# UWQuickstep/quickstep

Measured on AMD Instinct MI355X. Metric: probe+aggregate rows/s at TPC-H SF100 (Q1,Q3), higher is better.
Workload: dtype i32 keys / f64 sums

## Files before the change

quickstep_amd/capi.py:

```python
import ctypes as C
import os

import torch

from . import types as T

_HERE = os.path.dirname(os.path.abspath(__file__))
LIB_PATH = os.environ.get("QSX_LIB_PATH") or os.path.join(_HERE, "lib", "libqsx.so")


class QsxError(RuntimeError):
    def __init__(self, status, where):
        self.status = status
        msg = _lib.qsx_status_string(status).decode()
        detail = _lib.qsx_last_error().decode()
        super().__init__(f"{where}: {msg} ({status})" + (f" — {detail}" if detail and status in (T.ERR_HIP, T.ERR_COMM) else ""))


def _load():
    if not os.path.exists(LIB_PATH):
        raise ImportError(
            f"{LIB_PATH} is missing: build it with `python -c 'import __graft_entry__ as g; g.build()'` "
            "(or make -C quickstep_amd/csrc). There is no CPU fallback for the HIP execution kernel.")
    return C.CDLL(LIB_PATH)
# ... 120 lines not shown
    "qsx_agg_state_image_layout": (_int, [_vp, C.POINTER(_int), C.POINTER(_i64), C.POINTER(_i64), C.POINTER(_int), C.POINTER(_i32), _int]),
    "qsx_agg_state_import_merge": (_int, [_vp, _vp, _sz, _vp]),
    "qsx_agg_num_groups": (_int, [_vp, C.POINTER(_i64), _vp]),
    "qsx_agg_finalize": (_int, [_vp, _int, _int, _pp, _pp, _pp, _i64, _vp, _vp]),
    "qsx_lip_filter_create": (_int, [_int, _i64, _i64, _int, _pp]),
    "qsx_lip_filter_destroy": (_int, [_vp]),
    "qsx_lip_build": (_int, [_vp, _int, _vp, _i64, _vp, _vp]),
    "qsx_lip_build_from_join_table": (_int, [_vp, _vp, _i64, _vp]),
    "qsx_lip_probe": (_int, [_vp, _int, _vp, _i64, _vp, _vp, _vp, _vp]),
    "qsx_lip_build_blocks": (_int, [_vp, _int, _i64, C.POINTER(_i64), _pp, _pp, _vp]),
    "qsx_lip_probe_blocks": (_int, [_vp, _int, _i64, C.POINTER(_i64), _pp, _pp, _pp, _vp, _vp]),
    "qsx_lip_build_blocks_coded": (_int, [_vp, _int, _i64, C.POINTER(_i64), _pp, _vp, _pp, _vp]),
    "qsx_lip_probe_blocks_coded": (_int, [_vp, _int, _i64, C.POINTER(_i64), _pp, _vp, _pp, _pp, _vp, _vp]),
    "qsx_lip_filter_words": (_int, [_vp, _pp, C.POINTER(_i64)]),
    "qsx_comm_unique_id": (_int, [_vp]),
    "qsx_comm_create": (_int, [_int, _int, _vp, _pp]),
    "qsx_comm_destroy": (_int, [_vp]),
    "qsx_comm_rank": (_int, [_vp, C.POINTER(_int), C.POINTER(_int)]),
    "qsx_comm_agree": (_int, [_vp, _int, _vp]),
    "qsx_comm_synchronize": (_int, [_vp, _vp]),
    "qsx_comm_abort": (_int, [_vp]),
    "qsx_exchange_counts": (_int, [_vp, _vp, _vp, _vp]),
    "qsx_alltoallv": (_int, [_vp, _int, _vp, C.POINTER(_i64), _vp, C.POINTER(_i64), _vp]),
    "qsx_allgather": (_int, [_vp, _vp, _sz, _vp, _vp]),
    "qsx_bitmap_allreduce_or": (_int, [_vp, _vp, _i64, _vp]),
    "qsx_agg_reduce_scatter": (_int, [_vp, _vp, _vp]),
    "qsx_agg_allgather_merge": (_int, [_vp, _vp, _vp]),
    "qsx_agg_dense_partition_range": (_int, [_i64, _int, _int, C.POINTER(_i64), C.POINTER(_i64), C.POINTER(_i64), C.POINTER(_i64),
                                             C.POINTER(C.c_uint64), C.POINTER(C.c_uint64)]),
    "qsx_partition_workspace_bytes": (_sz, [_i64, _int]),
    "qsx_partition_scatter": (_int, [_int, _vp, _i64, _int, _int, _pp, C.POINTER(_i32), _pp, _vp, _vp, _sz, _vp]),
    "qsx_partition_blocks_workspace_bytes": (_sz, [_i64, _i64, _int]),
    "qsx_partition_scatter_blocks": (_int, [_int, _i64, C.POINTER(_i64), _pp, _int, _int, _pp, C.POINTER(_i32), _pp, _vp, _vp, _sz, _vp]),
}

for _name, (_res, _args) in _SIGNATURES.items():
    _fn = getattr(_lib, _name)
    _fn.restype = _res
    _fn.argtypes = _args

if _lib.qsx_abi_sizeof_agg_config() != C.sizeof(T.AggConfig):
    raise ImportError("quickstep_amd.types.AggConfig does not match qsx_agg_config_t of libqsx.so")

if _lib.qsx_abi_sizeof_sort_key() != C.sizeof(T.SortKey):
    raise ImportError("quickstep_amd.types.SortKey does not match qsx_sort_key_t of libqsx.so")

if _lib.qsx_abi_sizeof_case_desc() != C.sizeof(T.CaseDesc):
    raise ImportError("quickstep_amd.types.CaseDesc does not match qsx_case_desc_t of libqsx.so")

lib = _lib
EXPORTED = tuple(_SIGNATURES)


def _check(status, where):
    if status != T.OK:
        raise QsxError(status, where)


def trim_scratch():
    v = C.c_size_t()
    _check(_lib.qsx_trim_scratch(C.byref(v)), "qsx_trim_scratch")
    return v.value


def device_count():
    return _lib.qsx_device_count()


def current_device():
    v = C.c_int(-1)
    _check(_lib.qsx_current_device(C.byref(v)), "qsx_current_device")
    return v.value


def set_current_device(device):
    _check(_lib.qsx_set_current_device(int(device)), "qsx_set_current_device")


def _ptr(t):
    return None if t is None else C.c_void_p(t.data_ptr())


def _stream(stream=None):
    s = torch.cuda.current_stream() if stream is None else stream
    return C.c_void_p(s.cuda_stream)


_TORCH_TYPE = {torch.int32: T.INT, torch.int64: T.LONG, torch.float32: T.FLOAT, torch.float64: T.DOUBLE,
               torch.uint8: T.CHAR}
_C_SCALAR = {T.INT: C.c_int32, T.LONG: C.c_int64, T.FLOAT: C.c_float, T.DOUBLE: C.c_double}


def qsx_type_of(t):
    return _TORCH_TYPE[t.dtype]


def bitmap_words(n):
    return (n + 63) // 64


def new_bitmap(n, device):
    return torch.empty(max(bitmap_words(n), 1), dtype=torch.int64, device=device)


def _ptr_array(tensors):
    arr = (C.c_void_p * max(len(tensors), 1))()
# ... 1139 lines not shown
```

quickstep_amd/csrc/join.hip:

```cpp

#include "common.hpp"
#include "join_dense.hpp"
#include "join_lds.hpp"
#include "scan.hpp"

#include <atomic>
#include <cstdlib>
#include <vector>
#include <mutex>
#include <shared_mutex>
#include <type_traits>

namespace qsx {

constexpr int kJBlock = 256;
constexpr uint64_t kEmpty64 = ~0ull;
constexpr uint32_t kEmptyTid = 0xFFFFFFFFu;

struct alignas(16) LongEntry {
  int64_t key;
  uint32_t tid;
  uint32_t pad;
};

// ... 1202 lines not shown
  for (int64_t b = 0; b < num_blocks; ++b) {
    const int64_t last = base[b] + block_rows[b] - 1;
    for (int64_t seen = t->max_tid.load(); seen < last && !t->max_tid.compare_exchange_weak(seen, last);) {}
  }
  hipStream_t s = as_stream(stream);
  std::vector<long long> table;
  const long long groups = build_run_table(kBuildTile, num_blocks, block_rows, block_keys,
                                           reinterpret_cast<const void *const *>(block_filters), nullptr, base.data(), &table,
                                           coding != nullptr ? coding->block_code_width : nullptr,
                                           coding != nullptr ? coding->block_dictionaries : nullptr);
  if (groups < 0) return QSX_ERR_INVALID_ARGUMENT;
  const size_t bytes = table.size() * sizeof(long long);
  const long long *runs_dev = static_cast<const long long *>(staged_device_buffer(s, bytes));
  if (runs_dev == nullptr) return QSX_ERR_OUT_OF_MEMORY;
  rc = staged_upload(s, table.data(), bytes);
  if (rc != QSX_OK) return rc;
  std::shared_lock<std::shared_mutex> lock(t->mutex);
  if (t->dense) {
    const int dgrid = grid_for(groups, kDBlock / kWave);
    if (t->key_type == QSX_INT) {
      hipLaunchKernelGGL((dense_build_kernel<int32_t, true>), dim3(dgrid), dim3(kDBlock), 0, s, t->dense_view(),
                         static_cast<const int32_t *>(nullptr), total, 0, static_cast<const uint64_t *>(nullptr), t->entries_dev, runs_dev);
    } else {
      hipLaunchKernelGGL((dense_build_kernel<int64_t, true>), dim3(dgrid), dim3(kDBlock), 0, s, t->dense_view(),
                         static_cast<const int64_t *>(nullptr), total, 0, static_cast<const uint64_t *>(nullptr), t->entries_dev, runs_dev);
    }
  } else {
    const int grid = grid_for(groups, kJBlock / kWave);
    if (t->key_type == QSX_INT) {
      hipLaunchKernelGGL(build_runs_kernel<int32_t>, dim3(grid), dim3(kJBlock), 0, s, t->view(), runs_dev, t->entries_dev);
    } else {
      hipLaunchKernelGGL(build_runs_kernel<int64_t>, dim3(grid), dim3(kJBlock), 0, s, t->view(), runs_dev, t->entries_dev);
    }
  }
  QSX_CHECK_LAUNCH();
  mark_stream(t, s);
  return QSX_OK;
}

int qsx_join_build_blocks(qsx_join_table_t *t, int64_t num_blocks, const int64_t *block_rows, const void *const *block_keys,
                          const int32_t *block_base_tids, const uint64_t *const *block_filters, qsx_stream_t stream) {
  return join_build_blocks_impl(t, num_blocks, block_rows, block_keys, block_base_tids, block_filters, nullptr, stream);
}
int qsx_join_build_blocks_coded(qsx_join_table_t *t, int64_t num_blocks, const int64_t *block_rows, const void *const *block_keys,
                                const qsx_key_coding_t *coding, const int32_t *block_base_tids, const uint64_t *const *block_filters,
                                qsx_stream_t stream) {
  return join_build_blocks_impl(t, num_blocks, block_rows, block_keys, block_base_tids, block_filters, coding, stream);
}

}

static std::atomic<long long> g_compact_probes{0};
extern "C" long long qsx_debug_join_compact_probes(void) { return g_compact_probes.load(std::memory_order_relaxed); }
static bool lds_tables_enabled() {
  const char *e = getenv("QSX_JOIN_LDS");
  return e == nullptr || e[0] != '0';
}

static bool dense_two_pass(const uint64_t *filter) {
  const char *e = getenv("QSX_JOIN_TWO_PASS");
  if (e != nullptr && e[0] != '\0') return e[0] != '0';
  return filter != nullptr;
}

static void drop_cover(qsx_join_table *t) {
  std::lock_guard<std::mutex> lock(t->cover_mutex);
  t->cover_state = 0;
  t->cover_sig.clear();
}

constexpr int64_t kAdaptiveMinRows = 1 << 16;
static bool adaptive_enabled() {
  const char *e = getenv("QSX_JOIN_ADAPTIVE");
  return e == nullptr || e[0] != '0';
}

static bool sealed_pack(qsx_join_table *t, hipStream_t stream, unsigned long long *count_word = nullptr) {
  auto behind_the_pack = [&]() {
    if (t->pack_stream != stream && t->pack_event != nullptr && hipEventQuery(t->pack_event) != hipSuccess) {
      (void)hipGetLastError();
      (void)hipStreamWaitEvent(stream, t->pack_event, 0);
    }
  };
  int state = t->seal_state.load(std::memory_order_acquire);
  if (state == 2) {
    behind_the_pack();
    return false;
  }
  if (state != 0 || !adaptive_enabled()) return false;
  const uint64_t bytes4 = t->range * 4, bytes3 = t->range * 3;
  if (bytes4 <= (13ull << 18) || bytes3 > (36ull << 20) / 10 || t->max_tid.load() >= (1 << 23) - 2 || t->reserved >= (1 << 23) - 1) {
    return false;
  }
  std::lock_guard<std::mutex> lock(t->seal_mutex);
  state = t->seal_state.load(std::memory_order_acquire);
  if (state != 0) {
    if (state == 2) behind_the_pack();
    return false;
  }
  if (t->head3 == nullptr && device_malloc(&t->head3, static_cast<size_t>(bytes3) + 4) != hipSuccess) {
    (void)hipGetLastError();
    t->head3 = nullptr;
    t->seal_state.store(1, std::memory_order_release);
    return false;
  }
  if (t->pack_event == nullptr && hipEventCreateWithFlags(&t->pack_event, hipEventDisableTiming) != hipSuccess) {
// ... 159 lines not shown
    if (!ensure_scanned()) return nullptr;
    if (!compact_possible(t) || !read_control_words(t, stream, v, &any_key) || !seal_compact(t, v[2] != 0, stream) || !publish_seal(t, stream, 3)) {
      t->seal_state.store(1, std::memory_order_release);
    }
    return nullptr;
  }
  qsx_join_table *shadow = t->shadow;
  if (shadow != nullptr && (shadow->min_key != lo || shadow->range != span + 1 || shadow->ov_capacity < entries)) {
    (void)qsx_join_table_destroy(shadow);
    shadow = t->shadow = nullptr;
  }
  if (shadow == nullptr) {
    if (qsx_join_table_create_dense(t->key_type, lo, hi, 1, static_cast<int64_t>(entries), &shadow) != QSX_OK) {
      (void)hipGetLastError();
      return stays_hashed();
    }
    t->shadow = shadow;
  } else if (qsx_join_table_clear(shadow, reinterpret_cast<qsx_stream_t>(stream)) != QSX_OK) {
    return stays_hashed();
  }
  shadow->reserved = static_cast<int64_t>(entries);
  shadow->max_tid.store(t->max_tid.load());
  const TableView src = t->view();
  hipLaunchKernelGGL(dense_build_from_slots_kernel, dim3(grid_for(static_cast<int64_t>(src.num_slots()), kJBlock * 4)), dim3(kJBlock), 0, stream,
                     t->key_type == QSX_LONG ? 1 : 0, src, shadow->dense_view());
  if (hipGetLastError() != hipSuccess) return stays_hashed();
  if (seal_verify_enabled()) {
    int error = 0;
    if (hipStreamSynchronize(stream) != hipSuccess ||
        hipMemcpy(&error, shadow->entries_dev + 3, sizeof(error), hipMemcpyDeviceToHost) != hipSuccess || error != 0) {
      set_last_error("QSX_JOIN_SEAL_VERIFY: the shadow's build reported an error", hipErrorUnknown);
      return stays_hashed();
    }
  }
  if (!publish_seal(t, stream, 2)) return stays_hashed();
  return shadow;
}

template <int MODE, bool kRuns, bool kLds = true, int NLIP = 0>
static int launch_lds_dense_probe(qsx_join_table_t *t, const void *keys, int64_t n, int32_t probe_base_tid, const uint64_t *filter,
                                  int32_t *out_probe, int32_t *out_build, int64_t capacity, unsigned long long *count,
                                  uint64_t *out_bitmap, int anti, hipStream_t stream, const long long *runs_dev, int64_t tiles,
                                  const LipViews &lips = LipViews{}) {
  const size_t table_bytes = kLds ? ((static_cast<size_t>(t->range) * 4 + 15) & ~static_cast<size_t>(15)) : 0;
  auto launch = [&](auto key_tag) -> int {
    using KeyT = decltype(key_tag);
    auto kernel = &lds_dense_probe_kernel<KeyT, MODE, kRuns, kLds, NLIP>;
    if (table_bytes > 48 * 1024) {
      QSX_HIP_TRY(hipFuncSetAttribute(reinterpret_cast<const void *>(kernel), hipFuncAttributeMaxDynamicSharedMemorySize, 160 * 1024 - kLdsStaticBytes));
    }
    const int sub = kLds ? kLdsSub : kLdsSubGlobal, per_cu = kLds ? 1 : 2;
    const int64_t units = (tiles + sub - 1) / sub;
    const int grid = static_cast<int>(units < static_cast<int64_t>(per_cu) * kCUs ? units : static_cast<int64_t>(per_cu) * kCUs);
    hipLaunchKernelGGL(kernel, dim3(grid), dim3(kLdsBlock), table_bytes, stream, t->dense_view(), static_cast<const KeyT *>(keys), n, probe_base_tid,
                       filter, out_probe, out_build, capacity, count, out_bitmap, anti, runs_dev, lips);
    QSX_CHECK_LAUNCH();
    return QSX_OK;
  };
  return t->key_type == QSX_INT ? launch(int32_t{}) : launch(int64_t{});
}

static bool one_pass_enabled() {
  const char *e = getenv("QSX_JOIN_ONE_PASS");
  return e == nullptr || e[0] != '0';
}

template <int MODE, bool kRuns = false>
static int launch_probe(qsx_join_table_t *t, const void *keys, int64_t n, int32_t probe_base_tid,
                        const uint64_t *filter, int32_t *out_probe, int32_t *out_build,
                        int64_t capacity, int64_t *out_count, uint64_t *out_bitmap, int anti,
                        hipStream_t stream, const long long *runs_dev = nullptr, int64_t run_tiles = 0) {
  static_assert(kDenseTile == kProbeTile, "one run table serves both table kinds");
  if (!t->dense && n != 0) {
    qsx_join_table *shadow = sealed_shadow(t, stream, n);
    if (shadow != nullptr) {
      return launch_probe<MODE, kRuns>(shadow, keys, n, probe_base_tid, filter, out_probe, out_build, capacity, out_count, out_bitmap,
                                       anti, stream, runs_dev, run_tiles);
    }
    if (!t->scanned.load(std::memory_order_acquire)) {
      set_last_error("the scan in front of a hashed table's first probe could not be issued", hipErrorUnknown);
      return QSX_ERR_HIP;
    }
  }
  const bool zeroed = n != 0 && t->dense && sealed_pack(t, stream, reinterpret_cast<unsigned long long *>(out_count));
  if (out_count != nullptr && !zeroed) QSX_HIP_TRY(hipMemsetAsync(out_count, 0, sizeof(int64_t), stream));
  if (n == 0) return QSX_OK;
  std::shared_lock<std::shared_mutex> lock(t->mutex);
  if (t->dense) {
    const int64_t tiles = kRuns ? run_tiles : (n + kDenseTile - 1) / kDenseTile;
    const int64_t limit = 8 * kCUs;
    const int dgrid = static_cast<int>(tiles < limit ? tiles : limit);
    unsigned long long *dcount = reinterpret_cast<unsigned long long *>(out_count);
    if constexpr (MODE == 0 || MODE == 1 || MODE == 2) {
      const bool two_pass = MODE == 0 && dense_two_pass(filter);
      if (!two_pass && lds_tables_enabled() && t->range <= static_cast<uint64_t>(kLdsDenseMaxWords) && n >= 32 * static_cast<int64_t>(t->range) &&
          n >= (1 << 18)) {
        return launch_lds_dense_probe<MODE, kRuns>(t, keys, n, probe_base_tid, filter, out_probe, out_build, capacity, dcount, out_bitmap, anti,
                                                   stream, runs_dev, tiles);
      }
    }
    if constexpr (MODE == 0) {
      if (dense_two_pass(filter) && one_pass_enabled() && n >= (1 << 20)) {
        return launch_lds_dense_probe<0, kRuns, false>(t, keys, n, probe_base_tid, filter, out_probe, out_build, capacity, dcount, out_bitmap, anti,
                                                       stream, runs_dev, tiles);
      }
    }
    if (MODE == 0 && dense_two_pass(filter)) {
      const int64_t units = tiles * (kDBlock / kWave);
      CallScratch scratch(stream);
      const size_t bytes_counts = static_cast<size_t>(units) * 4, bytes_offsets = static_cast<size_t>(units + 1) * 8,
                   bytes_scan = scan_workspace_words(units) * 8;
      const int rc_scratch = scratch.reserve(CallScratch::padded(bytes_counts) + CallScratch::padded(bytes_offsets) + CallScratch::padded(bytes_scan));
      if (rc_scratch != QSX_OK) return rc_scratch;
      int32_t *unit_counts = static_cast<int32_t *>(scratch.take(bytes_counts));
      int64_t *unit_offsets = static_cast<int64_t *>(scratch.take(bytes_offsets)), *scan_ws = static_cast<int64_t *>(scratch.take(bytes_scan));
      if (t->key_type == QSX_INT) {
        hipLaunchKernelGGL((dense_probe_kernel<int32_t, 3, kRuns>), dim3(dgrid), dim3(kDBlock), 0, stream, t->dense_view(),
                           static_cast<const int32_t *>(keys), n, probe_base_tid, filter, out_probe, out_build, capacity,
                           dcount, out_bitmap, anti, unit_counts, unit_offsets, runs_dev);
      } else {
        hipLaunchKernelGGL((dense_probe_kernel<int64_t, 3, kRuns>), dim3(dgrid), dim3(kDBlock), 0, stream, t->dense_view(),
                           static_cast<const int64_t *>(keys), n, probe_base_tid, filter, out_probe, out_build, capacity,
                           dcount, out_bitmap, anti, unit_counts, unit_offsets, runs_dev);
      }
      QSX_CHECK_LAUNCH();
      QSX_HIP_TRY(launch_scan(unit_counts, units, unit_offsets, out_count, scan_ws, stream));
      if (t->key_type == QSX_INT) {
        hipLaunchKernelGGL((dense_probe_kernel<int32_t, 4, kRuns>), dim3(dgrid), dim3(kDBlock), 0, stream, t->dense_view(),
                           static_cast<const int32_t *>(keys), n, probe_base_tid, filter, out_probe, out_build, capacity,
                           dcount, out_bitmap, anti, unit_counts, unit_offsets, runs_dev);
      } else {
        hipLaunchKernelGGL((dense_probe_kernel<int64_t, 4, kRuns>), dim3(dgrid), dim3(kDBlock), 0, stream, t->dense_view(),
                           static_cast<const int64_t *>(keys), n, probe_base_tid, filter, out_probe, out_build, capacity,
                           dcount, out_bitmap, anti, unit_counts, unit_offsets, runs_dev);
      }
      QSX_CHECK_LAUNCH();
      return QSX_OK;
    }
    if (t->key_type == QSX_INT) {
      hipLaunchKernelGGL((dense_probe_kernel<int32_t, MODE, kRuns>), dim3(dgrid), dim3(kDBlock), 0, stream, t->dense_view(),
                         static_cast<const int32_t *>(keys), n, probe_base_tid, filter, out_probe, out_build, capacity,
                         dcount, out_bitmap, anti, nullptr, nullptr, runs_dev);
    } else {
      hipLaunchKernelGGL((dense_probe_kernel<int64_t, MODE, kRuns>), dim3(dgrid), dim3(kDBlock), 0, stream, t->dense_view(),
                         static_cast<const int64_t *>(keys), n, probe_base_tid, filter, out_probe, out_build, capacity,
                         dcount, out_bitmap, anti, nullptr, nullptr, runs_dev);
    }
    QSX_CHECK_LAUNCH();
    return QSX_OK;
  }
  const int64_t num_tiles = kRuns ? run_tiles : (n + kProbeTile - 1) / kProbeTile;
  if constexpr (MODE == 0 || MODE == 1 || MODE == 2) {
    if (lds_tables_enabled() && t->table_bytes() <= kLdsBucketMaxBytes && n >= (1 << 18) && n >= 8 * static_cast<int64_t>(t->capacity)) {
      const size_t table_bytes = (t->table_bytes() + 15) & ~static_cast<size_t>(15);
      auto launch = [&](auto key_tag) -> int {
        using KeyT = decltype(key_tag);
        auto kernel = &lds_bucket_probe_kernel<KeyT, MODE, kRuns>;
        if (table_bytes > 48 * 1024) {
          QSX_HIP_TRY(hipFuncSetAttribute(reinterpret_cast<const void *>(kernel), hipFuncAttributeMaxDynamicSharedMemorySize, 160 * 1024 - kLdsStaticBytes));
        }
        const int64_t units = (num_tiles + kLdsSub - 1) / kLdsSub;
        const int lgrid = static_cast<int>(units < kCUs ? units : kCUs);
        hipLaunchKernelGGL(kernel, dim3(lgrid), dim3(kLdsBlock), table_bytes, stream, t->view(), static_cast<const KeyT *>(keys), n, probe_base_tid, filter,
                           out_probe, out_build, capacity, reinterpret_cast<unsigned long long *>(out_count), out_bitmap, anti, runs_dev);
        QSX_CHECK_LAUNCH();
        return QSX_OK;
      };
      return t->key_type == QSX_INT ? launch(int32_t{}) : launch(int64_t{});
    }
  }
  const int64_t max_grid = MODE == 0 ? 4 * kCUs : 8 * kCUs;
  const int grid = static_cast<int>(num_tiles < max_grid ? num_tiles : max_grid);
  unsigned long long *count = reinterpret_cast<unsigned long long *>(out_count);
  if constexpr (MODE == 0 || MODE == 1 || MODE == 2) {
    if (t->key_type == QSX_INT && t->seal_state.load(std::memory_order_acquire) == 3 && compact_enabled()) {
      g_compact_probes.fetch_add(1, std::memory_order_relaxed);
      hipLaunchKernelGGL((probe_fp_kernel<int32_t, MODE, kRuns, true>), dim3(grid), dim3(kJBlock), 0, stream, t->view(),
                         static_cast<const int32_t *>(keys), n, probe_base_tid, filter, out_probe,
                         out_build, capacity, count, out_bitmap, anti, runs_dev, t->compact_view());
      QSX_CHECK_LAUNCH();
      return QSX_OK;
    }
  }
  if (t->key_type == QSX_INT) {
    hipLaunchKernelGGL((probe_fp_kernel<int32_t, MODE, kRuns>), dim3(grid), dim3(kJBlock), 0, stream, t->view(),
                       static_cast<const int32_t *>(keys), n, probe_base_tid, filter, out_probe,
                       out_build, capacity, count, out_bitmap, anti, runs_dev);
  } else {
    hipLaunchKernelGGL((probe_fp_kernel<int64_t, MODE, kRuns>), dim3(grid), dim3(kJBlock), 0, stream, t->view(),
                       static_cast<const int64_t *>(keys), n, probe_base_tid, filter, out_probe,
                       out_build, capacity, count, out_bitmap, anti, runs_dev);
  }
  QSX_CHECK_LAUNCH();
  return QSX_OK;
}

static int cover_for(qsx_join_table *t, const ProjectionView &view, int entry_bytes, bool wanted, const std::vector<long long> &signature,
// ... 352 lines not shown
    table[head_words + sg] = proj->build_first_tids[sg];
    signature.push_back(proj->build_first_tids[sg]);
    if (sg > 0) {
      const long long len = proj->build_first_tids[sg] - proj->build_first_tids[sg - 1];
      if (sg == 1) seg_rows = len;
      else if (len != seg_rows) seg_rows = -1;
    }
    for (int c = 0; c < nc; ++c) {
      if (proj->on_build[c] != 0) {
        table[head_words + nseg + static_cast<size_t>(sg) * nc + c] = word_of(proj->build_stripes[static_cast<size_t>(sg) * nc + c]);
        signature.push_back(table[head_words + nseg + static_cast<size_t>(sg) * nc + c]);
      }
    }
  }
  if (seg_rows <= 0 || seg_rows > INT32_MAX) seg_rows = 0;
  const int key_width = direct->key_type == QSX_INT ? 4 : 8;
  for (int c = 0; c < nc; ++c) table[static_cast<size_t>(4 * nc + c)] = proj->on_build[c] == 0 && proj->width[c] == key_width && num_blocks > 0 ? 1 : 0;
  for (int64_t b = 0; b < num_blocks; ++b) {
    for (int c = 0; c < nc; ++c) {
      if (proj->on_build[c] == 0) {
        const void *stripe = proj->probe_stripes[static_cast<size_t>(b) * nc + c];
        if (stripe == nullptr && block_rows[b] > 0) return QSX_ERR_INVALID_ARGUMENT;
        table[head_words + nseg + static_cast<size_t>(nseg) * nc + static_cast<size_t>(b) * nc + c] = word_of(stripe);
        if (block_rows[b] > 0 && stripe != block_keys[b]) table[static_cast<size_t>(4 * nc + c)] = 0;
      }
    }
  }
  const long long *runs_dev = nullptr, *proj_dev = nullptr;
  int64_t tiles = 0, rows = 0;
  bool any_filter = false;
  const int rc = upload_probe_run(num_blocks, block_rows, block_keys, nullptr, block_filters, nullptr, s, &runs_dev, &tiles, &rows,
                                  &any_filter, &table, &proj_dev, coding);
  if (rc != QSX_OK) return rc;
  QSX_HIP_TRY(hipMemsetAsync(out_count_dev, 0, sizeof(int64_t), s));
  if (rows == 0) return QSX_OK;
  sealed_pack(direct, s);
  ProjectionView view{proj_dev, nc, nseg, static_cast<int>(seg_rows), nullptr};
  const int cover_entry = cover_for(direct, view, cover_bytes, any_build && proj->num_build_segments > 0, signature, s, &view.cover);
  std::shared_lock<std::shared_mutex> lock(direct->mutex);
  const int64_t limit = 8 * kCUs;
  const int dgrid = static_cast<int>(tiles < limit ? tiles : limit);
  const uint64_t *filter_mark = any_filter ? reinterpret_cast<const uint64_t *>(runs_dev) : nullptr;
  unsigned long long *count = reinterpret_cast<unsigned long long *>(out_count_dev);
  const DenseTableView dv = direct->dense_view();
  constexpr int kCoverBlock = 512;
  const int cgrid = static_cast<int>(tiles < 4 * kCUs ? tiles : 4 * kCUs);
  auto by_entry = [&](auto key_tag) {
    using KeyT = decltype(key_tag);
    switch (cover_entry) {
      case 4: hipLaunchKernelGGL((cover_probe_kernel<KeyT, uint32_t, kCoverBlock>), dim3(cgrid), dim3(kCoverBlock), 0, s, dv, capacity, count, runs_dev, view); break;
      case 8: hipLaunchKernelGGL((cover_probe_kernel<KeyT, unsigned long long, kCoverBlock>), dim3(cgrid), dim3(kCoverBlock), 0, s, dv, capacity, count, runs_dev, view); break;
      case 16: hipLaunchKernelGGL((cover_probe_kernel<KeyT, ulonglong2, kCoverBlock>), dim3(cgrid), dim3(kCoverBlock), 0, s, dv, capacity, count, runs_dev, view); break;
      default:
        hipLaunchKernelGGL((dense_probe_kernel<KeyT, 5, true>), dim3(dgrid), dim3(kDBlock), 0, s, dv, static_cast<const KeyT *>(nullptr), rows, 0,
                           filter_mark, static_cast<int32_t *>(nullptr), static_cast<int32_t *>(nullptr), capacity, count,
                           static_cast<uint64_t *>(nullptr), 0, static_cast<int32_t *>(nullptr), static_cast<const int64_t *>(nullptr), runs_dev,
                           view);
        break;
    }
  };
  if (direct->key_type == QSX_INT) by_entry(int32_t{}); else by_entry(int64_t{});
  QSX_CHECK_LAUNCH();
  return QSX_OK;
}

static int join_probe_count_blocks_impl(qsx_join_table_t *t, int64_t num_blocks, const int64_t *block_rows, const void *const *block_keys,
                                const uint64_t *const *block_filters, int64_t *out_count_dev, const qsx_key_coding_t *coding, qsx_stream_t stream) {
  QSX_REQUIRE_DEVICE();
  if (t == nullptr || num_blocks < 0 || out_count_dev == nullptr || (num_blocks > 0 && (block_rows == nullptr || block_keys == nullptr))) {
    return QSX_ERR_INVALID_ARGUMENT;
  }
  hipStream_t s = as_stream(stream);
  const long long *runs_dev = nullptr;
  int64_t tiles = 0, rows = 0;
  bool any_filter = false;
  if (check_key_coding(&coding, num_blocks) != QSX_OK) return QSX_ERR_INVALID_ARGUMENT;
  const int rc = upload_probe_run(num_blocks, block_rows, block_keys, nullptr, block_filters, nullptr, s, &runs_dev, &tiles, &rows,
                                  &any_filter, nullptr, nullptr, coding);
  if (rc != QSX_OK) return rc;
  return launch_probe<1, true>(t, nullptr, rows, 0, nullptr, nullptr, nullptr, 0, out_count_dev, nullptr, 0, s, runs_dev, tiles);
}

static int join_probe_exists_blocks_impl(qsx_join_table_t *t, int64_t num_blocks, const int64_t *block_rows, const void *const *block_keys,
                                 const uint64_t *const *block_filters, int anti, uint64_t *const *block_out_bitmaps,
                                 int64_t *out_count_dev, const qsx_key_coding_t *coding, qsx_stream_t stream) {
  QSX_REQUIRE_DEVICE();
  if (t == nullptr || num_blocks < 0 ||
      (num_blocks > 0 && (block_rows == nullptr || block_keys == nullptr || block_out_bitmaps == nullptr))) {
    return QSX_ERR_INVALID_ARGUMENT;
  }
  hipStream_t s = as_stream(stream);
  const long long *runs_dev = nullptr;
  int64_t tiles = 0, rows = 0;
  bool any_filter = false;
  if (check_key_coding(&coding, num_blocks) != QSX_OK) return QSX_ERR_INVALID_ARGUMENT;
  const int rc = upload_probe_run(num_blocks, block_rows, block_keys, nullptr, block_filters, block_out_bitmaps, s, &runs_dev,
                                  &tiles, &rows, &any_filter, nullptr, nullptr, coding);
  if (rc != QSX_OK) return rc;
  return launch_probe<2, true>(t, nullptr, rows, 0, nullptr, nullptr, nullptr, 0, out_count_dev, nullptr, anti, s, runs_dev, tiles);
}

int qsx_join_probe_blocks(qsx_join_table_t *t, int64_t num_blocks, const int64_t *block_rows, const void *const *block_keys,
                          const int32_t *block_base_tids, const uint64_t *const *block_filters, int32_t *out_probe_tid_dev,
                          int32_t *out_build_tid_dev, int64_t capacity, int64_t *out_count_dev, qsx_stream_t stream) {
  return join_probe_blocks_impl(t, num_blocks, block_rows, block_keys, block_base_tids, block_filters, out_probe_tid_dev, out_build_tid_dev,
                                capacity, out_count_dev, nullptr, stream);
// ... 61 lines not shown
```

quickstep_amd/csrc/join_dense.hpp:

```cpp
#ifndef QSX_CSRC_JOIN_DENSE_HPP_
#define QSX_CSRC_JOIN_DENSE_HPP_

#include <type_traits>

#include "block_runs.hpp"
#include "common.hpp"

namespace qsx {

constexpr int kDBlock = 256;
constexpr int kDenseRowsPerThread = 16;
constexpr int kDenseTile = kDBlock * kDenseRowsPerThread;
constexpr uint32_t kChainBit = 0x80000000u;
constexpr int kDenseSparsePairs = 256;

struct DenseTableView {
  uint32_t *head;
  const unsigned char *head3;
  uint2 *ov;
  int64_t min_key;
  int stride_shift;
  uint64_t range;
  unsigned int *ov_count;
  unsigned int ov_capacity;
  int *error;
};

template <typename KeyT>
__device__ __forceinline__ uint64_t dense_index(const DenseTableView &t, KeyT key) {
  const uint64_t d = static_cast<uint64_t>(static_cast<int64_t>(key) - t.min_key);
  const uint64_t idx = d >> t.stride_shift;
  return (idx << t.stride_shift) == d && idx < t.range ? idx : ~0ull;
}

__device__ __forceinline__ uint32_t dense_head_word(const DenseTableView &t, uint64_t idx) {
  if (t.head3 == nullptr) return t.head[idx];
  uint32_t w;
  __builtin_memcpy(&w, t.head3 + idx * 3, 4);
  return (w & 0x7FFFFFu) | ((w & 0x800000u) << 8);
}

__device__ __forceinline__ bool dense_row_in_filter(const uint64_t *filter, int64_t row) {
  return filter == nullptr || ((filter[row >> 6] >> (63 - (row & 63))) & 1u);
}

constexpr int kBuildR = 8;
constexpr int kBuildTile = kBuildR * kWave;
template <typename KeyT, bool kRuns = false>
__global__ __launch_bounds__(kDBlock) void dense_build_kernel(DenseTableView t, const KeyT *__restrict__ keys, int64_t n,
                                                             int32_t base_tid_arg, const uint64_t *__restrict__ filter,
                                                             unsigned long long *__restrict__ entries,
                                                             const long long *__restrict__ runs = nullptr) {
  constexpr int R = kBuildR;
  using Source = ProbeTileSource<KeyT>;
  const int lane = lane_id();
  const int64_t num_groups = kRuns ? runs[2] : (((n + 63) >> 6) + R - 1) / R;
  const int64_t wave = __builtin_amdgcn_readfirstlane(static_cast<int>(blockIdx.x * (kDBlock / kWave) + (threadIdx.x >> 6)));
  const int64_t num_waves = static_cast<int64_t>(gridDim.x) * (kDBlock / kWave);
  unsigned long long inserted = 0;
  KeyT key[R], next_key[R];
  uint64_t words = ~0ull, next_words = ~0ull;
  auto source_of = [&](int64_t group) {
    return probe_tile_source<KeyT, kBuildTile, kRuns>(runs, group, keys, n, base_tid_arg, filter, nullptr);
  };
  auto request = [&](const Source &src, KeyT (&k)[R], uint64_t &fw) {
    const int64_t sw0 = src.base >> 6;
    if (kRuns && src.code_width != 0) {
      coded_keys(src, k, [&](int r) {
        const int64_t row = ((sw0 + r) << 6) + lane;
        return row < src.n ? row : src.n - 1;
      });
    } else {
#pragma unroll
      for (int r = 0; r < R; ++r) {
        const int64_t row = ((sw0 + r) << 6) + lane;
        k[r] = load_global(&src.keys[row < src.n ? row : src.n - 1]);
      }
    }
    fw = ~0ull;
    if (src.filter != nullptr && lane < R && sw0 + lane < ((src.n + 63) >> 6)) fw = load_global(&src.filter[sw0 + lane]);
  };
  Source cur = Source(), next = Source();
  int64_t group = wave;
  if (group < num_groups) {
    cur = source_of(group);
    request(cur, key, words);
  }
  for (; group < num_groups; group += num_waves) {
    if (group + num_waves < num_groups) {
      next = source_of(group + num_waves);
      request(next, next_key, next_words);
    }
// ... 102 lines not shown
    }
    const char *src = p.on_build(c) ? projected_build_value(p, c, width, tid) : p.probe_stripe(tile.block, c) + static_cast<size_t>(probe_row) * width;
    store_value(p.out(c) + o * width, load_value(src, width), width);
  }
}

template <typename EntryT>
__global__ __launch_bounds__(kDBlock) void cover_build_kernel(DenseTableView t, ProjectionView p, EntryT *__restrict__ cover,
                                                             unsigned int *__restrict__ flags) {
  const uint64_t i = static_cast<uint64_t>(blockIdx.x) * kDBlock + threadIdx.x;
  if (i >= t.range) return;
  const uint32_t hw = t.head[i];
  unsigned long long words[2] = {~0ull, ~0ull};
  if (hw & kChainBit) {
    atomicOr(flags, 1u);
  } else if (hw != 0u) {
    words[0] = words[1] = 0ull;
    for (int c = 0; c < p.nc; ++c) {
      if (!p.on_build(c)) continue;
      const int width = p.width(c), off = p.cover_offset(c);
      const unsigned long long v = load_value(projected_build_value(p, c, width, hw - 1u), width);
      if (off < 8) words[0] |= v << (8 * off); else words[1] |= v << (8 * (off - 8));
    }
    const bool ones = sizeof(EntryT) == 4 ? static_cast<uint32_t>(words[0]) == ~0u
                                          : (sizeof(EntryT) == 8 ? words[0] == ~0ull : (words[0] & words[1]) == ~0ull);
    if (ones) atomicOr(flags, 2u);
  }
  if constexpr (sizeof(EntryT) == 4) {
    cover[i] = static_cast<uint32_t>(words[0]);
  } else if constexpr (sizeof(EntryT) == 8) {
    cover[i] = words[0];
  } else {
    cover[i] = EntryT{words[0], words[1]};
  }
}

__device__ __forceinline__ void dense_emit_direct(bool match, int32_t probe_tid, int32_t build_tid,
                                                  int32_t *__restrict__ out_probe, int32_t *__restrict__ out_build,
                                                  unsigned long long capacity, unsigned long long *out_count) {
  const uint64_t m = __ballot(match);
  if (m == 0) return;
  unsigned long long base = 0;
  if (lane_id() == __ffsll(static_cast<long long>(m)) - 1) {
    base = atomicAdd(out_count, static_cast<unsigned long long>(__popcll(m)));
  }
  base = __shfl(base, __ffsll(static_cast<long long>(m)) - 1, kWave);
  const unsigned long long o = base + rank_below(m);
  if (match && o < capacity) {
    __builtin_nontemporal_store(probe_tid, &out_probe[o]);
    __builtin_nontemporal_store(build_tid, &out_build[o]);
  }
}

template <typename KeyT, int MODE, bool kRuns = false>
__global__ __launch_bounds__(kDBlock) __attribute__((amdgpu_waves_per_eu(MODE == 5 ? 3 : 1))) void dense_probe_kernel(
    DenseTableView t, const KeyT *__restrict__ keys, int64_t n, int32_t probe_base_tid,
    const uint64_t *__restrict__ filter, int32_t *__restrict__ out_probe, int32_t *__restrict__ out_build,
    int64_t capacity_signed, unsigned long long *__restrict__ out_count, uint64_t *__restrict__ out_bitmap, int anti,
    int32_t *__restrict__ unit_counts = nullptr, const int64_t *__restrict__ unit_offsets = nullptr,
    const long long *__restrict__ runs = nullptr, ProjectionView proj = ProjectionView{}) {
  constexpr int R = kDenseRowsPerThread;
  constexpr bool kProject = MODE == 5;
  using Source = ProbeTileSource<KeyT>;
  const unsigned long long capacity = static_cast<unsigned long long>(capacity_signed);
  const int64_t num_tiles = kRuns ? runs[2] : (n + kDenseTile - 1) / kDenseTile;
  auto source_of = [&](int64_t tile) {
    return probe_tile_source<KeyT, kDenseTile, kRuns>(runs, tile, keys, n, probe_base_tid, filter, out_bitmap);
  };
  unsigned long long local_count = 0;
  __shared__ int2 s_sparse[(MODE == 0 || MODE == 4) ? kDBlock / kWave : 1][(MODE == 0 || MODE == 4) ? kDenseSparsePairs : 1];
  __shared__ int s_wave_total[2][kDBlock / kWave];
  __shared__ unsigned long long s_tile_base;
  int parity = 0;
  const int wave = threadIdx.x >> 6;

  const int lane = lane_id();
  KeyT key[R], next_key[R];
  uint64_t filter_words = ~0ull, next_filter_words = ~0ull;
  auto request = [&](const Source &src, KeyT (&k)[R], uint64_t &words) {
    if (kRuns && src.code_width != 0) {
      coded_keys(src, k, [&](int r) {
        const int64_t row = src.base + r * kDBlock + threadIdx.x;
        return row < src.n ? row : src.n - 1;
      });
    } else {
#pragma unroll
      for (int r = 0; r < R; ++r) {
        const int64_t row = src.base + r * kDBlock + threadIdx.x;
        k[r] = load_global_nt(&src.keys[row < src.n ? row : src.n - 1]);
      }
    }
    words = ~0ull;
    if (src.filter != nullptr && lane < R) {
      const int64_t w = (src.base >> 6) + lane * (kDBlock / kWave) + wave;
      if (w < ((src.n + 63) >> 6)) words = load_global(&src.filter[w]);
    }
  };
  Source cur = Source(), next = Source();
  if (static_cast<int64_t>(blockIdx.x) < num_tiles) {
    cur = source_of(blockIdx.x);
    request(cur, key, filter_words);
  }

  for (int64_t tile = blockIdx.x; tile < num_tiles; tile += gridDim.x, parity ^= 1) {
    if (tile + gridDim.x < num_tiles) {
      next = source_of(tile + gridDim.x);
      request(next, next_key, next_filter_words);
    }
    const int64_t tile_base = cur.base;
    const int64_t n_rows = cur.n;
    const int32_t base_tid = cur.base_tid;
    uint64_t *const tile_bitmap = cur.out_bitmap;
    const int tile_block = cur.block;
    const Source tile_src = cur;
    cur = next;
    uint32_t h[R];
    uint32_t live_mask = 0;
#pragma unroll
    for (int r = 0; r < R; ++r) {
      const int64_t row = tile_base + r * kDBlock + threadIdx.x;
      const uint64_t filter_word = __shfl(filter_words, r, kWave);
      const bool live = row < n_rows && msb_bit(filter_word, lane);
      live_mask |= live ? (1u << r) : 0u;
      const uint64_t idx = dense_index(t, key[r]);
      const bool lookup = live && idx != ~0ull;
      const uint32_t word = dense_head_word(t, lookup ? idx : 0);
      h[r] = lookup ? word : 0u;
    }
#pragma unroll
    for (int r = 0; r < R; ++r) key[r] = next_key[r];
    filter_words = next_filter_words;

    if (MODE == 2) {
      uint64_t mine = 0;
#pragma unroll
      for (int r = 0; r < R; ++r) {
        const bool bit = ((live_mask >> r) & 1u) && ((h[r] != 0u) != (anti != 0));
        const uint64_t word = msb_first(__ballot(bit));
        if (lane == r) mine = word;
        if (lane == 0) local_count += __popcll(word);
      }
      const int64_t w = (tile_base >> 6) + lane * (kDBlock / kWave) + wave;
      if (lane < R && w < ((n_rows + 63) >> 6)) store_global(mine, &tile_bitmap[w]);
      continue;
    }

    uint64_t m[R];
    int total = 0;
    bool any_chain = false;
#pragma unroll
    for (int r = 0; r < R; ++r) {
      m[r] = __ballot(h[r] != 0u);
      total += __popcll(m[r]);
      any_chain = any_chain || (h[r] & kChainBit) != 0u;
    }
    const bool wave_has_chain = __any(any_chain);
    uint32_t next[R];
    unsigned long long base = 0;
    if (MODE == 1 || MODE == 3) {
      if (lane == 0) local_count += total;
      if (wave_has_chain) {
#pragma unroll
        for (int r = 0; r < R; ++r) next[r] = (h[r] & kChainBit) ? t.ov[h[r] & ~kChainBit].y : 0u;
      }
    } else {
      if (MODE == 0 || kProject) {
        if (lane == 0) s_wave_total[parity][wave] = total;
        __syncthreads();
        if (threadIdx.x == 0) {
          int all = 0;
#pragma unroll
          for (int w = 0; w < kDBlock / kWave; ++w) all += s_wave_total[parity][w];
          s_tile_base = all != 0 ? atomicAdd(out_count, static_cast<unsigned long long>(all)) : 0ull;
        }
        __syncthreads();
        base = s_tile_base;
        for (int w = 0; w < wave; ++w) base += s_wave_total[parity][w];
      } else {
        base = static_cast<unsigned long long>(unit_offsets[tile * (kDBlock / kWave) + wave]);
      }
      const bool sparse = !kProject && total <= kDenseSparsePairs;
// ... 289 lines not shown
```

quickstep_amd/csrc/join_lds.hpp:

```cpp
#ifndef QSX_CSRC_JOIN_LDS_HPP_
#define QSX_CSRC_JOIN_LDS_HPP_

#include "join_dense.hpp"
#include "lip_view.hpp"

namespace qsx {

constexpr int kLdsTile = kDenseTile;
constexpr int kLdsDenseMaxWords = 36 * 1024;
constexpr int kLdsStaticBytes = 1024;

constexpr int kLdsBlock = 1024;
constexpr int kLdsSub = 4;
constexpr int kMaxFusedLip = 2;
struct LipViews {
  LipView f[kMaxFusedLip];
};
constexpr int kLdsSubGlobal = 2;
template <typename KeyT, int MODE, bool kRuns = false, bool kLds = true, int NLIP = 0>
__global__ __launch_bounds__(kLdsBlock, kLds ? 1 : 8) void lds_dense_probe_kernel(DenseTableView t, const KeyT *__restrict__ keys, int64_t n,
                                                                   int32_t probe_base_tid, const uint64_t *__restrict__ filter,
                                                                   int32_t *__restrict__ out_probe, int32_t *__restrict__ out_build,
                                                                   int64_t capacity_signed, unsigned long long *__restrict__ out_count,
                                                                   uint64_t *__restrict__ out_bitmap, int anti,
// ... 47 lines not shown
  };
  if (static_cast<int64_t>(blockIdx.x) < num_super) request(blockIdx.x, key, filter_words);
  if constexpr (kLds) {
    const int range = static_cast<int>(t.range);
    typedef unsigned int u32x4 __attribute__((ext_vector_type(4)));
    const u32x4 *src4 = reinterpret_cast<const u32x4 *>(t.head);
    for (int i = threadIdx.x; i < (range >> 2); i += BLOCK) {
      const u32x4 v = load_global(&src4[i]);
      reinterpret_cast<u32x4 *>(l_head)[i] = v;
    }
    for (int i = (range & ~3) + threadIdx.x; i < range; i += BLOCK) l_head[i] = load_global(&t.head[i]);
  }
  __syncthreads();

  unsigned long long local_count = 0;
  int parity = 0;
  for (int64_t super = blockIdx.x; super < num_super; super += gridDim.x, parity ^= 1) {
    if (super + gridDim.x < num_super) request(super + gridDim.x, next_key, next_filter_words);
    uint32_t h[S][R];
    uint32_t live_mask = 0;
#pragma unroll
    for (int s = 0; s < S; ++s) {
      const int64_t tile = super * S + s;
      const bool present = tile < num_tiles;
      const Source src = present ? source_of(tile) : Source();
      const int64_t n_rows = present ? src.n : 0;
      bool live[R];
#pragma unroll
      for (int r = 0; r < R; ++r) {
        const int64_t row = src.base + r * BLOCK + threadIdx.x;
        const uint64_t filter_word = __shfl(filter_words[s], r, kWave);
        live[r] = row < n_rows && msb_bit(filter_word, lane);
      }
      if constexpr (NLIP > 0) {
#pragma unroll
        for (int f = 0; f < NLIP; ++f) {
          long long bit[R];
          unsigned long long w[R];
#pragma unroll
          for (int r = 0; r < R; ++r) {
            bit[r] = live[r] ? lip_bit_index(lips.f[f], static_cast<long long>(key[s][r])) : -2;
            w[r] = load_global(&lips.f[f].words[bit[r] >= 0 ? bit[r] >> 6 : 0]);
          }
#pragma unroll
          for (int r = 0; r < R; ++r) {
            const bool set = bit[r] >= 0 && ((w[r] >> (bit[r] & 63)) & 1ull) != 0;
            live[r] = live[r] && (bit[r] == -1 ? lips.f[f].is_anti != 0 : (set != (lips.f[f].is_anti != 0)));
          }
        }
      }
#pragma unroll
      for (int r = 0; r < R; ++r) {
        live_mask |= live[r] ? (1u << (s * R + r)) : 0u;
        const uint64_t idx = dense_index(t, key[s][r]);
        const bool lookup = live[r] && idx != ~0ull;
        uint32_t word;
        if constexpr (kLds) word = l_head[lookup ? static_cast<int>(idx) : 0];
        else word = dense_head_word(t, lookup ? idx : 0);
        h[s][r] = lookup ? word : 0u;
      }
    }
#pragma unroll
    for (int s = 0; s < S; ++s) {
#pragma unroll
      for (int r = 0; r < R; ++r) key[s][r] = next_key[s][r];
      filter_words[s] = next_filter_words[s];
    }

    if (MODE == 2) {
#pragma unroll
      for (int s = 0; s < S; ++s) {
        const int64_t tile = super * S + s;
        if (tile >= num_tiles) break;
        const Source src = source_of(tile);
        uint64_t mine = 0;
#pragma unroll
        for (int r = 0; r < R; ++r) {
          const bool bit = ((live_mask >> (s * R + r)) & 1u) && ((h[s][r] != 0u) != (anti != 0));
          const uint64_t word = msb_first(__ballot(bit));
          if (lane == r) mine = word;
          if (lane == 0) local_count += __popcll(word);
        }
        const int64_t w = (src.base >> 6) + lane * kWaves + wave;
        if (lane < R && w < ((src.n + 63) >> 6)) store_global(mine, &src.out_bitmap[w]);
      }
      continue;
    }

    uint64_t m[S][R];
    int total = 0;
    bool any_chain = false;
#pragma unroll
    for (int s = 0; s < S; ++s) {
#pragma unroll
      for (int r = 0; r < R; ++r) {
        m[s][r] = __ballot(h[s][r] != 0u);
        total += __popcll(m[s][r]);
        any_chain = any_chain || (h[s][r] & kChainBit) != 0u;
      }
    }
    const bool wave_has_chain = __any(any_chain);
    uint32_t chain_next[S][R];
    if (MODE == 1) {
      if (lane == 0) local_count += total;
      if (wave_has_chain) {
#pragma unroll
        for (int s = 0; s < S; ++s) {
#pragma unroll
          for (int r = 0; r < R; ++r) chain_next[s][r] = (h[s][r] & kChainBit) ? t.ov[h[s][r] & ~kChainBit].y : 0u;
        }
      }
    } else {
      if (lane == 0) s_wave_total[parity][wave] = total;
      __syncthreads();
// ... 71 lines not shown
```

Baseline: 190.5 billion.

## Batch dense head-word gathers and issue next-tile key prefetch behind them

Replaces the per-row head-word lookup with a batched helper that issues all gather loads first, then runs a callback (the next tile's key/filter prefetch), then decodes the packed 3-byte words. In the dense probe kernel this overlaps the next tile's key loads with the outstanding table gathers and removes the branch around the prefetch. The filter-word load is made branchless with a dummy address, and the waves-per-EU occupancy hint rises to 3–4 for most variants. It also adds a debug counter for packed-table probes. Higher occupancy hints may cap registers and spill, and the unconditional prefetch reloads the current tile on the last iteration.

```diff
diff --git a/quickstep_amd/capi.py b/quickstep_amd/capi.py
--- a/quickstep_amd/capi.py
+++ b/quickstep_amd/capi.py
@@ -196,6 +196,13 @@
 EXPORTED = tuple(_SIGNATURES)
 
 
+
+def join_packed_probes():
+    fn = _lib.qsx_debug_join_packed_probes
+    fn.restype, fn.argtypes = C.c_longlong, []
+    return fn()
+
+
 def _check(status, where):
     if status != T.OK:
         raise QsxError(status, where)
diff --git a/quickstep_amd/csrc/join.hip b/quickstep_amd/csrc/join.hip
--- a/quickstep_amd/csrc/join.hip
+++ b/quickstep_amd/csrc/join.hip
@@ -1278,6 +1278,13 @@
 
 static std::atomic<long long> g_compact_probes{0};
 extern "C" long long qsx_debug_join_compact_probes(void) { return g_compact_probes.load(std::memory_order_relaxed); }
+static std::atomic<long long> g_packed_probes{0};
+extern "C" long long qsx_debug_join_packed_probes(void) { return g_packed_probes.load(std::memory_order_relaxed); }
+static DenseTableView probe_view(const qsx_join_table *t) {
+  const DenseTableView v = t->dense_view();
+  if (v.head3 != nullptr) g_packed_probes.fetch_add(1, std::memory_order_relaxed);
+  return v;
+}
 static bool lds_tables_enabled() {
   const char *e = getenv("QSX_JOIN_LDS");
   return e == nullptr || e[0] != '0';
@@ -1543,7 +1550,7 @@
     const int sub = kLds ? kLdsSub : kLdsSubGlobal, per_cu = kLds ? 1 : 2;
     const int64_t units = (tiles + sub - 1) / sub;
     const int grid = static_cast<int>(units < static_cast<int64_t>(per_cu) * kCUs ? units : static_cast<int64_t>(per_cu) * kCUs);
-    hipLaunchKernelGGL(kernel, dim3(grid), dim3(kLdsBlock), table_bytes, stream, t->dense_view(), static_cast<const KeyT *>(keys), n, probe_base_tid,
+    hipLaunchKernelGGL(kernel, dim3(grid), dim3(kLdsBlock), table_bytes, stream, kLds ? t->dense_view() : probe_view(t), static_cast<const KeyT *>(keys), n, probe_base_tid,
                        filter, out_probe, out_build, capacity, count, out_bitmap, anti, runs_dev, lips);
     QSX_CHECK_LAUNCH();
     return QSX_OK;
@@ -1606,22 +1613,22 @@
       int32_t *unit_counts = static_cast<int32_t *>(scratch.take(bytes_counts));
       int64_t *unit_offsets = static_cast<int64_t *>(scratch.take(bytes_offsets)), *scan_ws = static_cast<int64_t *>(scratch.take(bytes_scan));
       if (t->key_type == QSX_INT) {
-        hipLaunchKernelGGL((dense_probe_kernel<int32_t, 3, kRuns>), dim3(dgrid), dim3(kDBlock), 0, stream, t->dense_view(),
+        hipLaunchKernelGGL((dense_probe_kernel<int32_t, 3, kRuns>), dim3(dgrid), dim3(kDBlock), 0, stream, probe_view(t),
                            static_cast<const int32_t *>(keys), n, probe_base_tid, filter, out_probe, out_build, capacity,
                            dcount, out_bitmap, anti, unit_counts, unit_offsets, runs_dev);
       } else {
-        hipLaunchKernelGGL((dense_probe_kernel<int64_t, 3, kRuns>), dim3(dgrid), dim3(kDBlock), 0, stream, t->dense_view(),
+        hipLaunchKernelGGL((dense_probe_kernel<int64_t, 3, kRuns>), dim3(dgrid), dim3(kDBlock), 0, stream, probe_view(t),
                            static_cast<const int64_t *>(keys), n, probe_base_tid, filter, out_probe, out_build, capacity,
                            dcount, out_bitmap, anti, unit_counts, unit_offsets, runs_dev);
       }
       QSX_CHECK_LAUNCH();
       QSX_HIP_TRY(launch_scan(unit_counts, units, unit_offsets, out_count, scan_ws, stream));
       if (t->key_type == QSX_INT) {
-        hipLaunchKernelGGL((dense_probe_kernel<int32_t, 4, kRuns>), dim3(dgrid), dim3(kDBlock), 0, stream, t->dense_view(),
+        hipLaunchKernelGGL((dense_probe_kernel<int32_t, 4, kRuns>), dim3(dgrid), dim3(kDBlock), 0, stream, probe_view(t),
                            static_cast<const int32_t *>(keys), n, probe_base_tid, filter, out_probe, out_build, capacity,
                            dcount, out_bitmap, anti, unit_counts, unit_offsets, runs_dev);
       } else {
-        hipLaunchKernelGGL((dense_probe_kernel<int64_t, 4, kRuns>), dim3(dgrid), dim3(kDBlock), 0, stream, t->dense_view(),
+        hipLaunchKernelGGL((dense_probe_kernel<int64_t, 4, kRuns>), dim3(dgrid), dim3(kDBlock), 0, stream, probe_view(t),
                            static_cast<const int64_t *>(keys), n, probe_base_tid, filter, out_probe, out_build, capacity,
                            dcount, out_bitmap, anti, unit_counts, unit_offsets, runs_dev);
       }
@@ -1629,11 +1636,11 @@
       return QSX_OK;
     }
     if (t->key_type == QSX_INT) {
-      hipLaunchKernelGGL((dense_probe_kernel<int32_t, MODE, kRuns>), dim3(dgrid), dim3(kDBlock), 0, stream, t->dense_view(),
+      hipLaunchKernelGGL((dense_probe_kernel<int32_t, MODE, kRuns>), dim3(dgrid), dim3(kDBlock), 0, stream, probe_view(t),
                          static_cast<const int32_t *>(keys), n, probe_base_tid, filter, out_probe, out_build, capacity,
                          dcount, out_bitmap, anti, nullptr, nullptr, runs_dev);
     } else {
-      hipLaunchKernelGGL((dense_probe_kernel<int64_t, MODE, kRuns>), dim3(dgrid), dim3(kDBlock), 0, stream, t->dense_view(),
+      hipLaunchKernelGGL((dense_probe_kernel<int64_t, MODE, kRuns>), dim3(dgrid), dim3(kDBlock), 0, stream, probe_view(t),
                          static_cast<const int64_t *>(keys), n, probe_base_tid, filter, out_probe, out_build, capacity,
                          dcount, out_bitmap, anti, nullptr, nullptr, runs_dev);
     }
@@ -2092,6 +2099,7 @@
       case 8: hipLaunchKernelGGL((cover_probe_kernel<KeyT, unsigned long long, kCoverBlock>), dim3(cgrid), dim3(kCoverBlock), 0, s, dv, capacity, count, runs_dev, view); break;
       case 16: hipLaunchKernelGGL((cover_probe_kernel<KeyT, ulonglong2, kCoverBlock>), dim3(cgrid), dim3(kCoverBlock), 0, s, dv, capacity, count, runs_dev, view); break;
       default:
+        if (dv.head3 != nullptr) g_packed_probes.fetch_add(1, std::memory_order_relaxed);
         hipLaunchKernelGGL((dense_probe_kernel<KeyT, 5, true>), dim3(dgrid), dim3(kDBlock), 0, s, dv, static_cast<const KeyT *>(nullptr), rows, 0,
                            filter_mark, static_cast<int32_t *>(nullptr), static_cast<int32_t *>(nullptr), capacity, count,
                            static_cast<uint64_t *>(nullptr), 0, static_cast<int32_t *>(nullptr), static_cast<const int64_t *>(nullptr), runs_dev,
diff --git a/quickstep_amd/csrc/join_dense.hpp b/quickstep_amd/csrc/join_dense.hpp
--- a/quickstep_amd/csrc/join_dense.hpp
+++ b/quickstep_amd/csrc/join_dense.hpp
@@ -33,11 +33,40 @@
   return (idx << t.stride_shift) == d && idx < t.range ? idx : ~0ull;
 }
 
-__device__ __forceinline__ uint32_t dense_head_word(const DenseTableView &t, uint64_t idx) {
-  if (t.head3 == nullptr) return t.head[idx];
-  uint32_t w;
-  __builtin_memcpy(&w, t.head3 + idx * 3, 4);
-  return (w & 0x7FFFFFu) | ((w & 0x800000u) << 8);
+struct NothingBehindReads {
+  __device__ __forceinline__ void operator()() const {}
+};
+template <typename KeyT, int N, typename Between = NothingBehindReads>
+__device__ __forceinline__ void dense_head_words(const DenseTableView &t, const KeyT *key, uint32_t live_mask, uint32_t *h,
+                                                 Between behind_reads = Between()) {
+  const bool packed = t.head3 != nullptr;
+  uint32_t lookup_mask = 0;
+  uint32_t w[N];
+  if (packed) {
+#pragma unroll
+    for (int i = 0; i < N; ++i) {
+      const uint64_t idx = dense_index(t, key[i]);
+      const bool lookup = ((live_mask >> i) & 1u) && idx != ~0ull;
+      lookup_mask |= lookup ? (1u << i) : 0u;
+      const uint32_t off = lookup ? static_cast<uint32_t>(idx) * 3u : 0u;
+      __builtin_memcpy(&w[i], t.head3 + off, 4);
+    }
+  } else {
+#pragma unroll
+    for (int i = 0; i < N; ++i) {
+      const uint64_t idx = dense_index(t, key[i]);
+      const bool lookup = ((live_mask >> i) & 1u) && idx != ~0ull;
+      lookup_mask |= lookup ? (1u << i) : 0u;
+      w[i] = t.head[lookup ? idx : 0];
+    }
+  }
+  behind_reads();
+  if (packed) {
+#pragma unroll
+    for (int i = 0; i < N; ++i) w[i] = (w[i] & 0x7FFFFFu) | ((w[i] & 0x800000u) << 8);
+  }
+#pragma unroll
+  for (int i = 0; i < N; ++i) h[i] = ((lookup_mask >> i) & 1u) ? w[i] : 0u;
 }
 
 __device__ __forceinline__ bool dense_row_in_filter(const uint64_t *filter, int64_t row) {
@@ -246,8 +275,10 @@
   }
 }
 
+template <typename KeyT, int MODE, bool kRuns>
+constexpr int kDenseProbeWaves = MODE == 5 || kRuns || sizeof(KeyT) == 8 ? 3 : 4;
 template <typename KeyT, int MODE, bool kRuns = false>
-__global__ __launch_bounds__(kDBlock) __attribute__((amdgpu_waves_per_eu(MODE == 5 ? 3 : 1))) void dense_probe_kernel(
+__global__ __launch_bounds__(kDBlock) __attribute__((amdgpu_waves_per_eu(kDenseProbeWaves<KeyT, MODE, kRuns>))) void dense_probe_kernel(
     DenseTableView t, const KeyT *__restrict__ keys, int64_t n, int32_t probe_base_tid,
     const uint64_t *__restrict__ filter, int32_t *__restrict__ out_probe, int32_t *__restrict__ out_build,
     int64_t capacity_signed, unsigned long long *__restrict__ out_count, uint64_t *__restrict__ out_bitmap, int anti,
@@ -271,6 +302,9 @@
   const int lane = lane_id();
   KeyT key[R], next_key[R];
   uint64_t filter_words = ~0ull, next_filter_words = ~0ull;
+  auto has_filter_word = [&](const Source &src) {
+    return src.filter != nullptr && lane < R && (src.base >> 6) + lane * (kDBlock / kWave) + wave < ((src.n + 63) >> 6);
+  };
   auto request = [&](const Source &src, KeyT (&k)[R], uint64_t &words) {
     if (kRuns && src.code_width != 0) {
       coded_keys(src, k, [&](int r) {
@@ -278,17 +312,16 @@
         return row < src.n ? row : src.n - 1;
       });
     } else {
+      const int tile_rows = static_cast<int>(src.n - src.base < kDenseTile ? src.n - src.base : kDenseTile);
+      const KeyT *tile_keys = src.keys + src.base;
 #pragma unroll
       for (int r = 0; r < R; ++r) {
-        const int64_t row = src.base + r * kDBlock + threadIdx.x;
-        k[r] = load_global_nt(&src.keys[row < src.n ? row : src.n - 1]);
-      }
-    }
-    words = ~0ull;
-    if (src.filter != nullptr && lane < R) {
-      const int64_t w = (src.base >> 6) + lane * (kDBlock / kWave) + wave;
-      if (w < ((src.n + 63) >> 6)) words = load_global(&src.filter[w]);
-    }
+        const int in_tile = r * kDBlock + static_cast<int>(threadIdx.x);
+        k[r] = load_global_nt(&tile_keys[in_tile < tile_rows ? in_tile : tile_rows - 1]);
+      }
+    }
+    const int64_t w = (src.base >> 6) + lane * (kDBlock / kWave) + wave;
+    words = load_global(has_filter_word(src) ? &src.filter[w] : reinterpret_cast<const uint64_t *>(t.ov_count));
   };
   Source cur = Source(), next = Source();
   if (static_cast<int64_t>(blockIdx.x) < num_tiles) {
@@ -297,30 +330,25 @@
   }
 
   for (int64_t tile = blockIdx.x; tile < num_tiles; tile += gridDim.x, parity ^= 1) {
-    if (tile + gridDim.x < num_tiles) {
-      next = source_of(tile + gridDim.x);
-      request(next, next_key, next_filter_words);
-    }
+    next = source_of(tile + gridDim.x < num_tiles ? tile + gridDim.x : tile);
     const int64_t tile_base = cur.base;
     const int64_t n_rows = cur.n;
     const int32_t base_tid = cur.base_tid;
     uint64_t *const tile_bitmap = cur.out_bitmap;
     const int tile_block = cur.block;
     const Source tile_src = cur;
+    if (!has_filter_word(cur)) filter_words = ~0ull;
     cur = next;
     uint32_t h[R];
     uint32_t live_mask = 0;
+    const int tile_rows = static_cast<int>(n_rows - tile_base < kDenseTile ? n_rows - tile_base : kDenseTile);
 #pragma unroll
     for (int r = 0; r < R; ++r) {
-      const int64_t row = tile_base + r * kDBlock + threadIdx.x;
       const uint64_t filter_word = __shfl(filter_words, r, kWave);
-      const bool live = row < n_rows && msb_bit(filter_word, lane);
+      const bool live = r * kDBlock + static_cast<int>(threadIdx.x) < tile_rows && msb_bit(filter_word, lane);
       live_mask |= live ? (1u << r) : 0u;
-      const uint64_t idx = dense_index(t, key[r]);
-      const bool lookup = live && idx != ~0ull;
-      const uint32_t word = dense_head_word(t, lookup ? idx : 0);
-      h[r] = lookup ? word : 0u;
-    }
+    }
+    dense_head_words<KeyT, R>(t, key, live_mask, h, [&]() __attribute__((always_inline)) { request(next, next_key, next_filter_words); });
 #pragma unroll
     for (int r = 0; r < R; ++r) key[r] = next_key[r];
     filter_words = next_filter_words;
diff --git a/quickstep_amd/csrc/join_lds.hpp b/quickstep_amd/csrc/join_lds.hpp
--- a/quickstep_amd/csrc/join_lds.hpp
+++ b/quickstep_amd/csrc/join_lds.hpp
@@ -123,14 +123,16 @@
 #pragma unroll
       for (int r = 0; r < R; ++r) {
         live_mask |= live[r] ? (1u << (s * R + r)) : 0u;
-        const uint64_t idx = dense_index(t, key[s][r]);
-        const bool lookup = live[r] && idx != ~0ull;
-        uint32_t word;
-        if constexpr (kLds) word = l_head[lookup ? static_cast<int>(idx) : 0];
-        else word = dense_head_word(t, lookup ? idx : 0);
-        h[s][r] = lookup ? word : 0u;
-      }
-    }
+        if constexpr (kLds) {
+          const uint64_t idx = dense_index(t, key[s][r]);
+          const bool lookup = live[r] && idx != ~0ull;
+          const uint32_t word = l_head[lookup ? static_cast<int>(idx) : 0];
+          h[s][r] = lookup ? word : 0u;
+        }
+      }
+      if constexpr (!kLds && NLIP > 0) dense_head_words<KeyT, R>(t, key[s], live_mask >> (s * R), h[s]);
+    }
+    if constexpr (!kLds && NLIP == 0) dense_head_words<KeyT, S * R>(t, &key[0][0], live_mask, &h[0][0]);
 #pragma unroll
     for (int s = 0; s < S; ++s) {
 #pragma unroll
```

New measurement: 190.3 billion. About the same (-0.1%).
